# huangzh13/StyleGAN.pytorch

Hardware: AMD Instinct MI355X
Metric: img/s full G+D train step, 1024x1024 depth-9 bf16 (higher is better)
Workload: dtype bf16; 1 GPU; ffhq1024: StyleGAN 1024x1024, progressive depth index 8, logistic+R1, alpha 0.5, batch 4/GPU, global batch 4; global_batch=4, parallelism=dp1

## Files before the change

### include/sgx.h

```cpp
#ifndef SGX_H
#define SGX_H
#include <stddef.h>
#include <stdint.h>
#ifdef __cplusplus
extern "C" {
#endif

enum { SGX_F32 = 0, SGX_BF16 = 1 };
enum { SGX_ACT_NONE = 0, SGX_ACT_LRELU = 1, SGX_ACT_RELU = 2 };
enum { SGX_EINVAL = -1, SGX_EUNSUPPORTED = -2, SGX_EWORKSPACE = -3 };

int sgx_version(void);
const char* sgx_last_error(void);
int sgx_clear_error(void);
int sgx_stream_wait_stream(void* waiter, void* signaler);
int sgx_selftest_tr16(void* out256, void* stream);

int sgx_prof_start(int mode, int only_of);
int sgx_prof_count(void);
int sgx_prof_get(int i, char* name, int name_cap, float* ms, double* flops, double* bytes, char* desc, int desc_cap);

int sgx_conv3x3(const void* x, const void* w, const float* bias, void* y, int B, int H, int W, int Cin, int Cout,
                int act, const void* mask, int dtype, void* stream);
int sgx_conv4x4s2_down(const void* x, const void* w, const float* bias, void* y, int B, int H, int W, int Cin,
// ... 126 lines not shown
int sgx_sumsq_f32(const float* x, size_t n, void* ws, size_t ws_bytes, float* out, void* stream);
int sgx_scale_dev_f32(const float* x, const float* s, float alpha, float* out, size_t n, void* stream);
int sgx_logistic_loss(const float* fake, int n_fake, const float* real, int n_real, float scale, int generator, float* loss,
                      float* g_fake, float* g_real, void* stream);
size_t sgx_gemm_ws_bytes(int M, int N, int K);
int sgx_gemm_f32(const float* A, const float* Bm, float* C, int M, int N, int K, int ta, int tb, float alpha,
                 void* ws, size_t ws_bytes, void* stream);
int sgx_linear_fwd(const float* x, const float* w, const float* bias, float* y, int B, int N, int K, float w_mul, float b_mul,
                   int act, void* stream);
int sgx_linear_bwd_data(const float* gy, const float* y_act, const float* w, float* gx, int B, int N, int K, float w_mul,
                        void* stream);
int sgx_linear_bwd_param(const float* gy, const float* y_act, const float* x, float* dw, float* db, int B, int N, int K, float w_mul,
                         float b_mul, void* stream);
#define SGX_STYLE_ROW 8
int sgx_style_fwd(const float* lm, const void* table, float* y, int G, int B, int D, int total_tiles, void* stream);
int sgx_style_bwd_data(const float* gy, const void* table, float* glm, int G, int B, int D, int max_n, void* stream);
int sgx_style_bwd_param(const float* gy, const float* lm, const void* table, float* dw, float* db, int G, int B, int D,
                        int total_tiles, void* stream);

int sgx_gepi_stats(const void* x, const float* bias, const float* noise, const float* nw, float* mean, float* rstd, void* ws, size_t ws_bytes,
                   const double* pre_part, int pre_npart, int B, int HW, int C, int flags, int dtype, void* stream);
int sgx_rgb_out_epi(const void* y, const float* ebias, const float* noise, const float* nw, const float* style, const float* mean,
                    const float* rstd, const float* w, int sj, int sc, float wscale, const float* rbias, const float* low, float alpha, float beta,
                    const float* ab_dev, float* img, int B, int H, int W, int C, int dtype, void* stream);
size_t sgx_rgb_wgrad_epi_ws_bytes(int B, int HW, int C);
int sgx_rgb_wgrad_epi(const void* y, const float* g, const float* ebias, const float* noise, const float* nw, const float* style, const float* mean,
                      const float* rstd, float* dw, float* db, int sj, int sc, float scale, float bscale, void* ws, size_t ws_bytes, int B, int HW,
                      int C, int dtype, void* stream);

int sgx_adam_multi(float* const* params, const float* const* grads, float* const* exp_avg, float* const* exp_avg_sq,
                   const int64_t* sizes, int n, float beta1, float beta2, float eps, const float* step_sizes,
                   const float* bc2_sqrts, const float* grad_scale, void* stream);
int sgx_ema_multi(float* const* tgt, const float* const* src, const int64_t* sizes, int n, float beta, void* stream);
int sgx_gradnorm_clip_coef(const float* const* grads, const int64_t* sizes, int n, float max_norm, double* partial,
                           float* out, void* stream);

#ifdef __cplusplus
}
#endif
#endif
```

### stylegan/pytorch_amd/GAN.py

```python
import contextlib
import copy
import datetime
import os
import random
import time
import timeit
from collections import OrderedDict

import numpy as np
import torch
import torch.nn as nn

from . import Losses
from . import functional as F
from .Blocks import DiscriminatorBlock, DiscriminatorTop, GSynthesisBlock, InputBlock
from .CustomLayers import EqualizedConv2d, EqualizedLinear, PixelNormLayer, Truncation, act_code, apply_act
from .data import get_data_loader
from . import native
from .native import ACT_LRELU
from .optim import FusedAdam, clip_and_step, ema_update


class DeferredLoss:

    __slots__ = ("_host", "_event", "_scale", "_value", "__weakref__")

    def __init__(self, dev_scalar, scale=1.0, stream=None):
        self._scale, self._value = float(scale), None
        if dev_scalar.is_cuda:
            with torch.cuda.stream(stream) if stream is not None else contextlib.nullcontext():
                t = dev_scalar.detach().reshape(1).float()
                view, slot = native.RING.take(4)
                self._host = view.view(torch.float32)
                self._host.copy_(t, non_blocking=True)
                self._event = native.RING.mark(slot, owner=self)
        else:
            self._host, self._event = dev_scalar.detach().reshape(1).float().clone(), None

    def item(self):
        if self._value is None:
            if self._event is not None:
                self._event.synchronize()
            self._value = float(self._host[0]) * self._scale
        return self._value

    __float__ = item

    def __format__(self, spec): return format(self.item(), spec)
    def __repr__(self): return repr(self.item())
    def __add__(self, o): return self.item() + float(o)
    __radd__ = __add__
    def __sub__(self, o): return self.item() - float(o)
    def __rsub__(self, o): return float(o) - self.item()
# ... 615 lines not shown
                loss.backward()
        except BaseException:
            self._sched_abort()
            raise
        if side is not None:
            torch.cuda.current_stream().wait_stream(side)
        self._note_active_grads("d", depth)
        return loss.detach()

    def _reduce(self, kind):
        if self.dp is None:
            return
        sched = self.__dict__.pop("_sched_active", None)
        if sched is not None and not sched.recording and sched.gb is not None and sched.gb.attached():
            try:
                sched.finish()
            except RuntimeError:
                for key in [k for k, v in self.__dict__.get("_bucket_scheds", {}).items() if v is sched]:
                    self._bucket_scheds.pop(key, None)
                    self._grad_buckets.pop(key, None)
                raise
            self.__dict__["_last_sched"] = sched
            return
        gb = next((g for (k, _), g in self._grad_buckets.items() if k == kind and g.attached()), None)
        if gb is not None:
            self.dp.all_reduce_buckets(gb)
        else:
            self.dp.all_reduce_grads((self.dis if kind == "d" else self.gen).parameters())

    def _d_reduce(self):
        self._reduce("d")

    def _d_update(self):
        self.dis_optim.step()

    def _g_grads(self, noise, real_batch, depth, alpha, labels=None):
        real_samples = None
        if not isinstance(self.loss, (Losses.LogisticGAN, Losses.HingeGAN, Losses.StandardGAN, Losses.ConditionalGANLoss)):
            real_samples = self.progressive_down_sampling(real_batch, depth, alpha)
        self._wait_update("g")
        fake_samples = self.gen(noise, depth, alpha, labels)
        self._wait_update("d")
        d_all = self.__dict__.get("_sgx_dis_params")
        if d_all is None:
            d_all = self.__dict__["_sgx_dis_params"] = list(self.dis.parameters())
        d_params = [p for p in d_all if p.requires_grad]
        for p in d_params:
            p.requires_grad_(False)
        try:
            if self.conditional:
                loss = self.loss.gen_loss(real_samples, fake_samples, labels, depth, alpha)
            else:
                loss = self.loss.gen_loss(real_samples, fake_samples, depth, alpha)
            self._zero_grads("g", depth)
            side = self._param_stream()
            self._sched_begin("g", depth, side)
            try:
                with F.accumulate_param_grads(), F.param_grad_stream(side):
                    loss.backward()
            except BaseException:
                self._sched_abort()
                raise
            if side is not None:
                torch.cuda.current_stream().wait_stream(side)
            self._note_active_grads("g", depth)
        finally:
            for p in d_params:
                p.requires_grad_(True)
        return loss.detach()

    def _g_reduce(self):
        self._reduce("g")

    def _g_update(self):
        clip_and_step(self.gen_optim, max_norm=10.)
        if self.use_ema:
            self.ema_updater(self.gen_shadow, self.gen, self.ema_decay)

    def _async_update(self, kind, loss):
        upd = self.__dict__.get("_update_stream")
        if upd is None:
            upd = self.__dict__["_update_stream"] = torch.cuda.Stream(device=self.device)
        upd.wait_stream(torch.cuda.current_stream())
        with torch.cuda.stream(upd):
            (self._d_reduce if kind == "d" else self._g_reduce)()
            loss.record_stream(upd)
            loss = self.dp.all_reduce_scalar(loss)
            (self._d_update if kind == "d" else self._g_update)()
        ev = torch.cuda.Event()
        ev.record(upd)
        self.__dict__.setdefault("_pending_updates", {})[kind] = ev
        self.__dict__["_loss_stream"] = upd
        return loss

    def _wait_update(self, kind):
        ev = self.__dict__.get("_pending_updates", {}).pop(kind, None)
        if ev is not None:
            torch.cuda.current_stream().wait_event(ev)

    def _d_body(self, noise, real_batch, depth, alpha, labels=None):
        loss = self._d_grads(noise, real_batch, depth, alpha, labels)
        if self.dp is not None and not torch.cuda.is_current_stream_capturing():
            return self._async_update("d", loss)
        self._d_reduce()
        self._d_update()
        return loss

    def _g_body(self, noise, real_batch, depth, alpha, labels=None):
        loss = self._g_grads(noise, real_batch, depth, alpha, labels)
# ... 205 lines not shown
                    torch.save(self.gen.state_dict(), gen_save_file)
                    logger.info("Saving the model to: %s\n" % gen_save_file)
                    torch.save(self.dis.state_dict(), os.path.join(save_dir, "GAN_DIS_" + tag))
                    torch.save(self.gen_optim.state_dict(), os.path.join(save_dir, "GAN_GEN_OPTIM_" + tag))
                    torch.save(self.dis_optim.state_dict(), os.path.join(save_dir, "GAN_DIS_OPTIM_" + tag))
                    if self.use_ema:
                        gen_shadow_save_file = os.path.join(save_dir, "GAN_GEN_SHADOW_" + tag)
                        torch.save(self.gen_shadow.state_dict(), gen_shadow_save_file)
                        logger.info("Saving the model to: %s\n" % gen_shadow_save_file)
        logger.info('Training completed.\n')



DP_EAGER_UPDATE = os.environ.get("SGX_DP_EAGER_UPDATE", "1") != "0"


class _StepGraph:

    WARMUP = 2

    def __init__(self, sg, kind, depth):
        self.sg, self.kind, self.depth = sg, kind, int(depth)
        self.calls = 0
        self.graph = None
        self.stream = torch.cuda.Stream(device=sg.device)
        self.z = self.real = self.loss = None
        dev = sg.device
        self.ab = torch.zeros(2, dtype=torch.float32, device=dev)
        self.ab_host = torch.zeros(2, dtype=torch.float32).pin_memory()
        self.cutoff = torch.zeros(1, dtype=torch.int64, device=dev)
        self.cutoff_host = torch.zeros(1, dtype=torch.int64).pin_memory()
        self.latents2 = self.latents2_host = None
        self.adam_entries = []
        self.graph_update = None
        self.split = False
        self.done = torch.cuda.Event()

    def _mixing(self):
        gen = self.sg.gen
        return gen.training and gen.style_mixing_prob is not None and gen.style_mixing_prob > 0

    def _stage(self, noise, real_batch, alpha):
        if self.z is None:
            self.z = torch.empty_like(noise)
            self.real = torch.empty_like(real_batch)
            if self._mixing():
                self.latents2 = torch.empty_like(noise)
                self.latents2_host = torch.empty(noise.shape, dtype=noise.dtype).pin_memory()
        if self._mixing():
            l2, cut = self.sg.gen.draw_mixing_host(noise.shape, self.depth)
            native._host_copy(self.latents2_host, l2); self.cutoff_host[0] = cut
            self.latents2.copy_(self.latents2_host, non_blocking=True)
            self.cutoff.copy_(self.cutoff_host, non_blocking=True)
        self.ab_host[0] = float(alpha); self.ab_host[1] = 1.0 - float(alpha)
        self.ab.copy_(self.ab_host, non_blocking=True)
        self.z.copy_(noise); self.real.copy_(real_batch)

    def _body(self, part="all"):
        sg = self.sg
        if part == "update":
            return (sg._d_update if self.kind == "d" else sg._g_update)()
        sg.gen._mixing_override = (self.latents2, self.cutoff) if self._mixing() else None
        try:
            name = {"all": "_body", "grads": "_grads"}[part]
            return getattr(sg, "_" + self.kind + name)(self.z, self.real, self.depth, self.ab)
        finally:
# ... 14 lines not shown
            self._stage(noise, real_batch, alpha)
            loss_stream = None
            if self.graph is None and self.calls < self.WARMUP:
                loss = self._body()
                loss_stream = sg.__dict__.pop("_loss_stream", None)
            else:
                if self.graph is None:
                    err = None
                    try:
                        self._capture()
                    except Exception as e:
                        err = e
                        torch.cuda.synchronize()
                        native.lib().sgx_clear_error()
                    ok = err is None if sg.dp is None else sg.dp.all_ok(err is None)
                    if not ok:
                        import sys
                        why = f"{type(err).__name__}: {err}" if err is not None else "it failed on another rank"
                        print(f"stylegan.pytorch_amd: hipGraph capture of the {self.kind}-step failed ({why}); "
                              "continuing eagerly", file=sys.stderr)
                        self.graph = self.graph_update = None
                        self.split = False
                        sg.use_graphs = False
                        torch.cuda.synchronize()
                        self._undo_failed_capture()
                        loss = self._body()
                        out = DeferredLoss(loss, stream=sg.__dict__.pop("_loss_stream", None))
                        self.done.record()
                        self.calls += 1
                        cur.wait_stream(self.stream)
                        return out
                else:
                    FusedAdam.graph_advance(self.adam_entries)
                self.graph.replay()
                if self.split:
                    for p, g in self.grads:
                        if p.grad is not g:
                            p.grad = g
                    (sg._d_reduce if self.kind == "d" else sg._g_reduce)()
                    self.loss_global = sg.dp.all_reduce_scalar(self.loss)
                    if self.graph_update is not None:
                        self.graph_update.replay()
                    else:
                        self._body("update")
                F.bump_weight_generation(self._changed_params())
                for p, g in self.grads:
                    if p.grad is not g:
                        p.grad = g
                loss = self.loss_global if self.split else self.loss
            out = DeferredLoss(loss, stream=loss_stream)
            self.done.record()
        self.calls += 1
        cur.wait_stream(self.stream)
        return out

    def _undo_failed_capture(self):
        F.clear_pack_cache()
        for st, val in self.__dict__.pop("_adam_steps_before_capture", []):
            st["step"] = torch.tensor(val)
        sg = self.sg
        nets = [sg.dis] if self.kind == "d" else [sg.gen]
        for net in nets:
            for p in net.parameters():
                p.grad = None
        self.adam_entries = []

    def _capture(self):
        sg = self.sg
        opt = sg.dis_optim if self.kind == "d" else sg.gen_optim
        opt.ensure_state()
        self._adam_steps_before_capture = [(st, float(st["step"])) for st in opt.state.values() if "step" in st]
        native.reserve_capture_staging(1 << 20)
        F.clear_pack_cache()
        import gc
        gc_was = False
        split = sg.dp is not None
        net = sg.dis if self.kind == "d" else sg.gen
        try:
            if os.environ.get("SGX_CAPTURE_GC_GUARD", "1") != "0":
                gc.collect()
                gc_was = gc.isenabled()
                gc.disable()
            torch.cuda.synchronize()
            opt._capture_log = []
            self.graph = torch.cuda.CUDAGraph()
            with torch.cuda.graph(self.graph, stream=self.stream, capture_error_mode="relaxed"):
                self.loss = self._body("grads" if split else "all")
            self.split = split
            if split and DP_EAGER_UPDATE:
                pass
            elif split:
                self.graph_update = torch.cuda.CUDAGraph()
                with torch.cuda.graph(self.graph_update, stream=self.stream, capture_error_mode="relaxed"):
                    self._body("update")
        finally:
            self.adam_entries, opt._capture_log = (getattr(opt, "_capture_log", None) or []), None
            if gc_was:
                gc.enable()
        self.grads = [(p, p.grad) for p in net.parameters() if p.grad is not None]
```

### stylegan/pytorch_amd/functional.py

```python
import contextlib
import functools
import os
import weakref

import numpy as np
import torch
from torch.autograd import Function
from torch.autograd.function import once_differentiable

from . import native as N

_DATA_GRAD_ONLY = 0


@contextlib.contextmanager
def data_grad_only():
    global _DATA_GRAD_ONLY
    _DATA_GRAD_ONLY += 1
    try:
        yield
    finally:
        _DATA_GRAD_ONLY -= 1


# ... 138 lines not shown
    mode, _, ipad, dtype = sub
    taps = 9 if mode == "S" else 16
    O = weight.shape[0]
    return (torch.empty((taps, O, ipad), dtype=dtype, device=weight.device), torch.empty((taps, ipad, O), dtype=dtype, device=weight.device))


def _pack_mark():
    ev = torch.cuda.Event()
    ev.record()
    raw = N.stream()
    return (ev, raw, {raw})


def prepack(weights):
    rows, blk, dtype, touched = [], 0, None, []
    for w in weights:
        ent = _PACKS.get(id(w))
        if ent is None or ent[0]() is not w or not ent[3]:
            continue
        tag = _pack_tag(w)
        if ent[1] == tag:
            continue
        if w.dtype != torch.float32 or not w.is_contiguous():
            raise N.SgxError("parameters must be contiguous fp32")
        ent[1], ent[2] = tag, {}
        touched.append(ent)
        for sub in ent[3]:
            if dtype is None:
                dtype = sub[3]
            if sub[3] != dtype:
                continue
            fwd, adj = _pack_alloc(w, sub)
            ent[2][sub] = (fwd, adj)
            O, I = w.shape[0], w.shape[1]
            nb = ((O + 31) // 32) * ((sub[2] + 31) // 32)
            rows.append([w.data_ptr(), fwd.data_ptr(), adj.data_ptr(), O, I, sub[2], MODES[sub[0]],
                         int(np.float32(sub[1]).view(np.uint32)), blk, nb])
            blk += nb
    if rows:
        table, _ = N.upload(torch.tensor(rows, dtype=torch.int64), weights[0].device)
        N.check(N.lib().sgx_pack_weight_multi(N.ptr(table), len(rows), blk, N.F32 if dtype == torch.float32 else N.BF16, N.stream()),
                "sgx_pack_weight_multi")
        if not N.capturing():
            table.record_stream(torch.cuda.current_stream())
        mark = _pack_mark()
        for ent in touched:
            ent[4] = mark


def packs(weight, mode, scale, ipad, dtype):
    key = id(weight)
    ent = _PACKS.get(key)
    tag = _pack_tag(weight)
    if ent is None or ent[0]() is not weight:
        ent = [weakref.ref(weight, lambda _r, k=key: _PACKS.pop(k, None)), tag, {}, set(), None]
        _PACKS[key] = ent
    elif ent[1] != tag:
        ent[1], ent[2] = tag, {}
    sub = (mode, float(scale), int(ipad), dtype)
    ent[3].add(sub)
    got = ent[2].get(sub)
    if got is not None and ent[4] is not None:
        raw = N.stream()
        if raw not in ent[4][2] or (not _FAST_FORK and raw != ent[4][1]):
            _stream_of(raw).wait_event(ent[4][0])
            ent[4][2].add(raw)
    if got is None:
        w = _c(weight.detach())
        if w.dtype != torch.float32:
            raise N.SgxError("parameters must be fp32")
        O, I = w.shape[0], w.shape[1]
        fwd, adj = _pack_alloc(w, sub)
        N.check(N.lib().sgx_pack_weight(N.ptr(w), N.ptr(fwd), N.ptr(adj), O, I, ipad, MODES[mode], float(scale),
                                        N.F32 if dtype == torch.float32 else N.BF16, N.stream()), "sgx_pack_weight")
        got = (fwd, adj)
        ent[2][sub] = got
        ent[4] = _pack_mark()
    return got


def clear_pack_cache():
    for ent in _PACKS.values():
        ent[1], ent[2] = None, {}
    _UPBLUR_PACKS.clear()


_UPBLUR_PACKS = {}


def upblur_pack(weight, mode, scale, ipad, adjoint):
    key = (id(weight), mode, float(scale), int(ipad), bool(adjoint))
    tag = _pack_tag(weight)
    ent = _UPBLUR_PACKS.get(key)
    if ent is not None and ent[0]() is weight and ent[1] == tag:
        raw = N.stream()
        if raw not in ent[3][2] or (not _FAST_FORK and raw != ent[3][1]):
            _stream_of(raw).wait_event(ent[3][0])
            ent[3][2].add(raw)
        return ent[2]
    w = _c(weight.detach())
    if w.dtype != torch.float32 or int(ipad) != w.shape[1]:
        raise N.SgxError("conv+blur composite pack: contiguous fp32 parameter without channel padding expected")
    O, I = w.shape[0], w.shape[1]
    Nn, K = (I, O) if adjoint else (O, I)
    wc = torch.empty(((9 * 4 + 22 * 2) * Nn * K,), dtype=torch.bfloat16, device=w.device)
    N.check(N.lib().sgx_pack_upblur(N.ptr(w), N.ptr(wc), O, I, MODES[mode], int(bool(adjoint)), float(scale) / 16.0, N.stream()), "sgx_pack_upblur")
    _UPBLUR_PACKS[key] = [weakref.ref(weight, lambda _r, k=key: _UPBLUR_PACKS.pop(k, None)), tag, wc, _pack_mark()]
    return wc


@functools.lru_cache(maxsize=None)
def _splitk_ws_bytes(gi, B, H, W, Cin, Cout, dt):
    return int(N.lib().sgx_conv_splitk_ws_bytes(gi, B, H, W, Cin, Cout, dt))


def _conv_launch(geo, x, wq, bias, act, mask=None):
    B, H, W, Cin = x.shape
# ... 1841 lines not shown
```

### stylegan/pytorch_amd/native.py

```python
import ctypes
import os
import subprocess
import threading

import torch

_HERE = os.path.dirname(os.path.abspath(__file__))
LIB_PATH = os.environ.get("SGX_HIP_LIB") or os.path.join(_HERE, "libsgx_hip.so")
CSRC = os.path.join(_HERE, "csrc")

F32, BF16 = 0, 1
ACT_NONE, ACT_LRELU, ACT_RELU = 0, 1, 2
EPI_ACT, EPI_NORM = 1, 2
PACK_S, PACK_D, PACK_U, PACK_UF = 0, 1, 2, 3

_lib = None
_lock = threading.Lock()

c_void_p, c_int, c_float, c_size_t = ctypes.c_void_p, ctypes.c_int, ctypes.c_float, ctypes.c_size_t
P, I, F, Z = c_void_p, c_int, c_float, c_size_t

SIGNATURES = {
    "sgx_version": (I, []),
    "sgx_last_error": (ctypes.c_char_p, []),
# ... 66 lines not shown
    "sgx_conv4x4s2_up_blur_bits": (I, [P, P, P, P, I, I, I, I, I, I, P]),
    "sgx_pack_upblur": (I, [P, P, I, I, I, I, F, P]),
    "sgx_conv_upblur_ok": (I, [I, I, I, I, I, I]),
    "sgx_conv_upblur": (I, [P, P, P, P, I, I, I, I, I, I, P]),
    "sgx_rgbconv_ok": (I, [I, I, I, I, I]),
    "sgx_rgbconv_pack": (I, [P, F, P, F, P, F, P, P, I, P]),
    "sgx_rgbconv_fwd": (I, [P, P, P, P, P, I, I, I, I, I, I, I, P]),
    "sgx_rgbconv_tune": (I, [I, I, I]),
    "sgx_rgbconv_dgrad": (I, [P, P, P, I, I, I, I, I, P]),
    "sgx_rgbconv_wgrad_ws_bytes": (Z, [I, I, I, I]),
    "sgx_rgbconv_wgrad": (I, [P, P, I, P, F, P, F, P, F, P, P, P, P, I, P, Z, I, I, I, I, I, P]),
    "sgx_conv3x3_stats": (I, [P, P, P, P, P, P, P, Z, I, I, I, I, I, I, P]),
    "sgx_blur3x3_stats": (I, [P, P, P, P, P, P, Z, I, I, I, I, I, I, P]),
    "sgx_gepi_bwd": (I, [P, P, P, P, P, P, P, P, P, P, P, P, P, Z, I, I, I, I, I, P]),
    "sgx_pixelnorm_fwd": (I, [P, P, I, I, P]),
    "sgx_pixelnorm_bwd": (I, [P, P, P, I, I, P]),
    "sgx_mbstd_fwd": (I, [P, P, I, I, I, I, I, P]),
    "sgx_mbstd_bwd": (I, [P, P, P, I, I, I, I, I, P]),
    "sgx_mbstd_bwd2": (I, [P, P, P, P, P, I, I, I, I, I, P]),
    "sgx_sumsq_ws_bytes": (Z, []),
    "sgx_sumsq_f32": (I, [P, Z, P, Z, P, P]),
    "sgx_scale_dev_f32": (I, [P, P, F, P, Z, P]),
    "sgx_logistic_loss": (I, [P, I, P, I, F, I, P, P, P, P]),
    "sgx_gemm_ws_bytes": (Z, [I, I, I]),
    "sgx_gemm_f32": (I, [P, P, P, I, I, I, I, I, F, P, Z, P]),
    "sgx_linear_fwd": (I, [P, P, P, P, I, I, I, F, F, I, P]),
    "sgx_linear_bwd_data": (I, [P, P, P, P, I, I, I, F, P]),
    "sgx_linear_bwd_param": (I, [P, P, P, P, P, I, I, I, F, F, P]),
    "sgx_style_fwd": (I, [P, P, P, I, I, I, I, P]),
    "sgx_style_bwd_data": (I, [P, P, P, I, I, I, I, P]),
    "sgx_style_bwd_param": (I, [P, P, P, P, P, I, I, I, I, P]),
    "sgx_adam_multi": (I, [P, P, P, P, P, I, F, F, F, P, P, P, P]),
    "sgx_ema_multi": (I, [P, P, P, I, F, P]),
    "sgx_gradnorm_clip_coef": (I, [P, P, I, F, P, P, P]),
}


def build(verbose: bool = False) -> str:
    cmd = ["make", "-C", CSRC, "-j", str(min(8, os.cpu_count() or 1))]
    r = subprocess.run(cmd, capture_output=True, text=True)
    if r.returncode != 0:
        raise RuntimeError("building libsgx_hip.so failed:\n" + r.stdout[-4000:] + r.stderr[-4000:])
    if verbose:
        print(r.stdout[-2000:])
    return LIB_PATH


def lib():
    global _lib
    if _lib is None:
        with _lock:
            if _lib is None:
                if not os.path.exists(LIB_PATH):
                    raise RuntimeError(f"{LIB_PATH} is missing: run `python -c 'import __graft_entry__ as g; g.build()'` "
                                       "(there is no non-HIP fallback for this path)")
                l = ctypes.CDLL(LIB_PATH)
                for name, (res, args) in SIGNATURES.items():
                    fn = getattr(l, name)
                    fn.restype, fn.argtypes = res, args
                _lib = l
    return _lib


class SgxError(RuntimeError):
    pass

# ... 180 lines not shown
```

### stylegan/pytorch_amd/optim.py

```python
import math
from collections import OrderedDict

import torch

from . import native as N
from .functional import bump_weight_generation


_TABLES = OrderedDict()
_TABLES_MAX = 64
_GRAPH_TABLES = []
_capturing = N.capturing
_to_dev = N.upload


def _dev_i64(vals, device):
    key = (tuple(vals), str(device))
    got = _TABLES.get(key)
    if got is None:
        got = _TABLES[key] = _to_dev(torch.tensor(vals, dtype=torch.int64), device)[0]
        while len(_TABLES) > _TABLES_MAX:
            _TABLES.popitem(last=False)
    else:
        _TABLES.move_to_end(key)
    if _capturing():
        _GRAPH_TABLES.append(got)
    elif got.is_cuda:
        got.record_stream(torch.cuda.current_stream())
    return got


def _dev_f32(vals, device):
    return _to_dev(torch.tensor(vals, dtype=torch.float32), device)


class FusedAdam(torch.optim.Optimizer):

    def __init__(self, params, lr=1e-3, betas=(0.9, 0.999), eps=1e-8):
        defaults = dict(lr=lr, betas=(float(betas[0]), float(betas[1])), eps=eps, weight_decay=0, amsgrad=False,
# ... 11 lines not shown
                    st["exp_avg"] = torch.zeros_like(p, memory_format=torch.preserve_format)
                    st["exp_avg_sq"] = torch.zeros_like(p, memory_format=torch.preserve_format)

    @staticmethod
    def _bias_scalars(act, lr, b1, b2):
        steps, bc2s = [], []
        for _, st in act:
            t = float(st["step"])
            steps.append(lr / (1.0 - b1 ** t))
            bc2s.append(math.sqrt(1.0 - b2 ** t))
        return steps + bc2s

    @staticmethod
    def graph_advance(entries):
        for pinned, act, group in entries:
            for _, st in act:
                st["step"] += 1
            b1, b2 = group["betas"]
            pinned.copy_(torch.tensor(FusedAdam._bias_scalars(act, group["lr"], b1, b2), dtype=torch.float32))

    def _active(self, group):
        out = []
        for p in group["params"]:
            if p.grad is None:
                continue
            st = self.state[p]
            if len(st) == 0:
                st["step"] = torch.tensor(0.0)
                st["exp_avg"] = torch.zeros_like(p, memory_format=torch.preserve_format)
                st["exp_avg_sq"] = torch.zeros_like(p, memory_format=torch.preserve_format)
            out.append((p, st))
        return out

    @torch.no_grad()
    def step(self, closure=None, grad_scale=None):
        assert closure is None
        L = N.lib()
        changed = []
        for group in self.param_groups:
            act = self._active(group)
            if not act:
                continue
            changed.extend(p for p, _ in act)
            b1, b2 = group["betas"]
            lr, eps = group["lr"], group["eps"]
            dev = act[0][0].device
            ptrs, sizes = [[], [], [], []], []
            for p, st in act:
                g = p.grad
                if not (p.is_contiguous() and g.is_contiguous() and p.dtype == torch.float32 and g.dtype == torch.float32):
                    raise N.SgxError("FusedAdam: parameters and gradients must be contiguous fp32")
                st["step"] += 1
                ptrs[0].append(p.data_ptr()); ptrs[1].append(g.data_ptr())
                ptrs[2].append(st["exp_avg"].data_ptr()); ptrs[3].append(st["exp_avg_sq"].data_ptr())
                sizes.append(p.numel())
            n = len(act)
            table = _dev_i64(ptrs[0] + ptrs[1] + ptrs[2] + ptrs[3] + sizes, dev)
            scal, pinned = _dev_f32(self._bias_scalars(act, lr, b1, b2), dev)
            if self._capture_log is not None and _capturing():
                self._capture_log.append((pinned, act, group))
            base, sb = table.data_ptr(), scal.data_ptr()
            N.check(L.sgx_adam_multi(base, base + 8 * n, base + 16 * n, base + 24 * n, base + 32 * n, n, b1, b2, eps,
                                     sb, sb + 4 * n, None if grad_scale is None else N.ptr(grad_scale), N.stream()),
                    "sgx_adam_multi")
            if not _capturing():
                scal.record_stream(torch.cuda.current_stream())
        bump_weight_generation(changed)
        return None


@torch.no_grad()
def clip_and_step(optim: FusedAdam, max_norm: float):
    L = N.lib()
    grads = [p.grad for g in optim.param_groups for p in g["params"] if p.grad is not None]
    if not grads:
        return
    dev = grads[0].device
    n = len(grads)
    table = _dev_i64([g.data_ptr() for g in grads] + [g.numel() for g in grads], dev)
    partial = torch.empty(n * 32, dtype=torch.float64, device=dev)
    out = torch.empty(2, dtype=torch.float32, device=dev)
    N.check(L.sgx_gradnorm_clip_coef(table.data_ptr(), table.data_ptr() + 8 * n, n, float(max_norm), N.ptr(partial),
                                     N.ptr(out), N.stream()), "sgx_gradnorm_clip_coef")
    optim.step(grad_scale=out[1:])
    return out


@torch.no_grad()
def ema_update(model_tgt, model_src, beta):
    pairs = model_tgt.__dict__.get("_sgx_ema_pairs")
    if pairs is None or pairs[0] != id(model_src):
        src = dict(model_src.named_parameters())
        pairs = model_tgt.__dict__["_sgx_ema_pairs"] = (id(model_src), [(p, src[name]) for name, p in model_tgt.named_parameters()])
    tg, sr, sizes = [], [], []
    dev = None
    changed = []
    for p, q in pairs[1]:
        changed.append(p)
        assert q is not p
        if not p.is_cuda:
            raise N.SgxError("ema_update needs GPU parameters")
        tg.append(p.data_ptr()); sr.append(q.data_ptr()); sizes.append(p.numel()); dev = p.device
        assert p.is_contiguous() and q.is_contiguous()
    n = len(tg)
    table = _dev_i64(tg + sr + sizes, dev)
    base = table.data_ptr()
    N.check(N.lib().sgx_ema_multi(base, base + 8 * n, base + 16 * n, n, float(beta), N.stream()), "sgx_ema_multi")
    bump_weight_generation(changed)
```

Measured before the change: 281.6 img/s.

## Fuse Adam update with conv weight repacking and EMA in one kernel

Adds a fused optimizer path that updates Adam state for 3x3 conv weights and writes the packed forward and adjoint bf16 weight layouts plus the EMA shadow in the same kernel. Non-conv parameters get a separate fused Adam+EMA kernel. Packed weight caches are kept across graph capture and marked rebuilt, so the next forward does not have to repack them. The aim is to cut the separate repack and EMA launches and the extra passes over weight memory, at the cost of more complex cache-invalidation logic around CUDA graph replay.

After: 283.5 img/s, median of 6. About the same (+0.7%).

```diff
diff --git a/include/sgx.h b/include/sgx.h
--- a/include/sgx.h
+++ b/include/sgx.h
@@ -182,6 +182,12 @@
                    const int64_t* sizes, int n, float beta1, float beta2, float eps, const float* step_sizes,
                    const float* bc2_sqrts, const float* grad_scale, void* stream);
 int sgx_ema_multi(float* const* tgt, const float* const* src, const int64_t* sizes, int n, float beta, void* stream);
+#define SGX_ADAM_PACK_ROW 14
+#define SGX_ADAM_EMA_ROW 6
+int sgx_adam_pack_multi(const void* table, int n, int total_blocks, int dtype, float beta1, float beta2, float eps,
+                        const float* step_sizes, const float* bc2_sqrts, const float* grad_scale, float ema_beta, void* stream);
+int sgx_adam_ema_multi(const void* table, int n, float beta1, float beta2, float eps, const float* step_sizes,
+                       const float* bc2_sqrts, const float* grad_scale, float ema_beta, void* stream);
 int sgx_gradnorm_clip_coef(const float* const* grads, const int64_t* sizes, int n, float max_norm, double* partial,
                            float* out, void* stream);
 
diff --git a/stylegan/pytorch_amd/GAN.py b/stylegan/pytorch_amd/GAN.py
--- a/stylegan/pytorch_amd/GAN.py
+++ b/stylegan/pytorch_amd/GAN.py
@@ -18,7 +18,8 @@
 from .data import get_data_loader
 from . import native
 from .native import ACT_LRELU
-from .optim import FusedAdam, clip_and_step, ema_update
+from . import optim as _optim
+from .optim import FusedAdam, clip_and_step, ema_pairs, ema_update
 
 
 class DeferredLoss:
@@ -700,6 +701,7 @@
         self._reduce("d")
 
     def _d_update(self):
+        self.dis_optim.attach(packed=_conv_weights(self.dis))
         self.dis_optim.step()
 
     def _g_grads(self, noise, real_batch, depth, alpha, labels=None):
@@ -741,8 +743,10 @@
         self._reduce("g")
 
     def _g_update(self):
+        fused_ema = self.use_ema and _optim.FUSED_OPT and self.ema_updater is update_average
+        self.gen_optim.attach(packed=_conv_weights(self.gen), ema=(ema_pairs(self.gen_shadow, self.gen), self.ema_decay) if fused_ema else None)
         clip_and_step(self.gen_optim, max_norm=10.)
-        if self.use_ema:
+        if self.use_ema and not fused_ema:
             self.ema_updater(self.gen_shadow, self.gen, self.ema_decay)
 
     def _async_update(self, kind, loss):
@@ -1014,6 +1018,7 @@
         self.cutoff_host = torch.zeros(1, dtype=torch.int64).pin_memory()
         self.latents2 = self.latents2_host = None
         self.adam_entries = []
+        self.pack_deps = []
         self.graph_update = None
         self.split = False
         self.done = torch.cuda.Event()
@@ -1094,6 +1099,7 @@
                         return out
                 else:
                     FusedAdam.graph_advance(self.adam_entries)
+                F.restore_packs(self.pack_deps)
                 self.graph.replay()
                 if self.split:
                     for p, g in self.grads:
@@ -1106,6 +1112,7 @@
                     else:
                         self._body("update")
                 F.bump_weight_generation(self._changed_params())
+                F.packs_replayed(self.pack_deps)
                 for p, g in self.grads:
                     if p.grad is not g:
                         p.grad = g
@@ -1118,6 +1125,7 @@
 
     def _undo_failed_capture(self):
         F.clear_pack_cache()
+        self.pack_deps = []
         for st, val in self.__dict__.pop("_adam_steps_before_capture", []):
             st["step"] = torch.tensor(val)
         sg = self.sg
@@ -1133,7 +1141,7 @@
         opt.ensure_state()
         self._adam_steps_before_capture = [(st, float(st["step"])) for st in opt.state.values() if "step" in st]
         native.reserve_capture_staging(1 << 20)
-        F.clear_pack_cache()
+        self.pack_deps = F.clear_pack_cache(_conv_weights(sg.gen) + _conv_weights(sg.dis) if _optim.FUSED_OPT else ())
         import gc
         gc_was = False
         split = sg.dp is not None
diff --git a/stylegan/pytorch_amd/csrc/optim_pack.hip b/stylegan/pytorch_amd/csrc/optim_pack.hip
--- /dev/null
+++ b/stylegan/pytorch_amd/csrc/optim_pack.hip
@@ -0,0 +1,232 @@
+#include "common.h"
+
+__device__ __forceinline__ float adam_one(float pi, float g, float& m, float& v, float gs, float beta1, float beta2, float eps, float step_size,
+                                          float bc2_sqrt) {
+    const float gi = g * gs;
+    const float mi = beta1 * m + (1.f - beta1) * gi;
+    const float vi = beta2 * v + (1.f - beta2) * gi * gi;
+    m = mi; v = vi;
+    const float denom = sqrtf(vi) / bc2_sqrt + eps;
+    return pi - step_size * (mi / denom);
+}
+__device__ __forceinline__ float ema_one(float a, float b, float beta) { return beta * a + (1.f - beta) * b; }
+
+#define PACK_T 32
+__device__ __forceinline__ float pack_tap(const float (*raw)[PACK_T][PACK_T + 1], int r, int il, int t, int mode, float scale) {
+    if (mode == SGX_PACK_S) return scale * raw[t][r][il];
+    const int ky = t >> 2, kx = t & 3;
+    float v = 0.f;
+#pragma unroll
+    for (int a = 0; a < 2; ++a)
+#pragma unroll
+        for (int b = 0; b < 2; ++b) {
+            const int y = ky - a, x = kx - b;
+            if (y >= 0 && y < 3 && x >= 0 && x < 3) v += raw[mode == SGX_PACK_UF ? (2 - y) * 3 + (2 - x) : y * 3 + x][r][il];
+        }
+    return v * scale * (mode == SGX_PACK_D ? 0.25f : 1.f);
+}
+
+struct AdamArgs { float beta1, beta2, eps, ema_beta; };
+
+template <typename T>
+__device__ __forceinline__ void adam_pack_tile(const long long* __restrict__ row, unsigned tile, AdamArgs a, float step_size, float bc2_sqrt,
+                                               float gs) {
+    __shared__ float raw[9][PACK_T][PACK_T + 1];
+    float* __restrict__ w = reinterpret_cast<float*>(row[0]);
+    T* __restrict__ fwd = reinterpret_cast<T*>(row[1]);
+    T* __restrict__ adj = reinterpret_cast<T*>(row[2]);
+    const int O = (int)row[3], I = (int)row[4], Ip = (int)row[5], mode = (int)row[6];
+    const float scale = __uint_as_float((unsigned)row[7]);
+    const float* __restrict__ g = reinterpret_cast<const float*>(row[10]);
+    float* __restrict__ m = reinterpret_cast<float*>(row[11]);
+    float* __restrict__ v = reinterpret_cast<float*>(row[12]);
+    float* __restrict__ sh = reinterpret_cast<float*>(row[13]);
+    const int tiles_i = (Ip + PACK_T - 1) / PACK_T;
+    const int o0 = (int)(tile / tiles_i) * PACK_T, i0 = (int)(tile % tiles_i) * PACK_T;
+    const int ni = (I - i0 < PACK_T ? (I - i0 > 0 ? I - i0 : 0) : PACK_T);
+    const bool aligned = ((row[0] | row[10] | row[11] | row[12] | row[13]) & 15) == 0;
+    if (ni == PACK_T && (I * 9) % 4 == 0 && ((size_t)i0 * 9) % 4 == 0 && aligned) {
+        constexpr int PER = PACK_T * (PACK_T * 9 / 4) / 256;
+        static_assert(PER * 256 == PACK_T * (PACK_T * 9 / 4), "a tile is a whole number of 16-byte accesses per thread");
+        float4 pw[PER], pg[PER], pm[PER], pv[PER], ps[PER];
+#pragma unroll
+        for (int u = 0; u < PER; ++u) {
+            const int idx = threadIdx.x + u * 256, r = idx / (PACK_T * 9 / 4), c4 = (idx % (PACK_T * 9 / 4)) * 4;
+            const size_t at = ((size_t)(o0 + r < O ? o0 + r : O - 1) * I + i0) * 9 + c4;
+            pw[u] = *reinterpret_cast<const float4*>(w + at);
+            pg[u] = *reinterpret_cast<const float4*>(g + at);
+            pm[u] = *reinterpret_cast<const float4*>(m + at);
+            pv[u] = *reinterpret_cast<const float4*>(v + at);
+            if (sh) ps[u] = *reinterpret_cast<const float4*>(sh + at);
+        }
+#pragma unroll
+        for (int u = 0; u < PER; ++u) {
+            const int idx = threadIdx.x + u * 256, r = idx / (PACK_T * 9 / 4), c4 = (idx % (PACK_T * 9 / 4)) * 4;
+            const bool ok = o0 + r < O;
+            float e[4] = {pw[u].x, pw[u].y, pw[u].z, pw[u].w};
+            const float eg[4] = {pg[u].x, pg[u].y, pg[u].z, pg[u].w};
+            float em[4] = {pm[u].x, pm[u].y, pm[u].z, pm[u].w};
+            float ev[4] = {pv[u].x, pv[u].y, pv[u].z, pv[u].w};
+#pragma unroll
+            for (int j = 0; j < 4; ++j) e[j] = adam_one(e[j], eg[j], em[j], ev[j], gs, a.beta1, a.beta2, a.eps, step_size, bc2_sqrt);
+            if (ok) {
+                const size_t at = ((size_t)(o0 + r) * I + i0) * 9 + c4;
+                *reinterpret_cast<float4*>(w + at) = make_float4(e[0], e[1], e[2], e[3]);
+                *reinterpret_cast<float4*>(m + at) = make_float4(em[0], em[1], em[2], em[3]);
+                *reinterpret_cast<float4*>(v + at) = make_float4(ev[0], ev[1], ev[2], ev[3]);
+                if (sh) {
+                    const float es[4] = {ps[u].x, ps[u].y, ps[u].z, ps[u].w};
+                    *reinterpret_cast<float4*>(sh + at) = make_float4(ema_one(es[0], e[0], a.ema_beta), ema_one(es[1], e[1], a.ema_beta),
+                                                                      ema_one(es[2], e[2], a.ema_beta), ema_one(es[3], e[3], a.ema_beta));
+                }
+            }
+#pragma unroll
+            for (int j = 0; j < 4; ++j) raw[(c4 + j) % 9][r][(c4 + j) / 9] = ok ? e[j] : 0.f;
+        }
+    } else
+    for (int idx = threadIdx.x; idx < PACK_T * PACK_T * 9; idx += blockDim.x) {
+        const int r = idx / (PACK_T * 9), c = idx % (PACK_T * 9);
+        const int il = c / 9, k = c % 9;
+        float pn = 0.f;
+        if (o0 + r < O && il < ni) {
+            const size_t at = ((size_t)(o0 + r) * I + i0) * 9 + c;
+            float mi = m[at], vi = v[at];
+            pn = adam_one(w[at], g[at], mi, vi, gs, a.beta1, a.beta2, a.eps, step_size, bc2_sqrt);
+            w[at] = pn; m[at] = mi; v[at] = vi;
+            if (sh) sh[at] = ema_one(sh[at], pn, a.ema_beta);
+        }
+        raw[k][r][il] = pn;
+    }
+    __syncthreads();
+    const int taps = mode == SGX_PACK_S ? 9 : 16;
+    constexpr int VE = 16 / (int)sizeof(T), VPR = PACK_T / VE;
+    const bool full = (o0 + PACK_T <= O) && (i0 + PACK_T <= Ip) && (O % VE == 0) && (Ip % VE == 0);
+    if (full) {
+        for (int e = threadIdx.x; e < taps * PACK_T * VPR; e += blockDim.x) {
+            const int t = e / (PACK_T * VPR), r = (e / VPR) % PACK_T, vv = e % VPR;
+            float val[VE];
+#pragma unroll
+            for (int j = 0; j < VE; ++j) val[j] = pack_tap(raw, r, vv * VE + j, t, mode, scale);
+            VecTraits<T>::store(fwd + ((size_t)t * O + o0 + r) * Ip + i0 + vv * VE, val);
+        }
+        for (int e = threadIdx.x; e < taps * PACK_T * VPR; e += blockDim.x) {
+            const int t = e / (PACK_T * VPR), il = (e / VPR) % PACK_T, vv = e % VPR;
+            const int ta = mode == SGX_PACK_S ? 8 - t : t;
+            float val[VE];
+#pragma unroll
+            for (int j = 0; j < VE; ++j) val[j] = pack_tap(raw, vv * VE + j, il, t, mode, scale);
+            VecTraits<T>::store(adj + ((size_t)ta * Ip + i0 + il) * O + o0 + vv * VE, val);
+        }
+        return;
+    }
+    for (int e = threadIdx.x; e < taps * PACK_T * PACK_T; e += blockDim.x) {
+        const int t = e / (PACK_T * PACK_T), r = (e / PACK_T) % PACK_T, il = e % PACK_T;
+        if (o0 + r < O && i0 + il < Ip)
+            fwd[((size_t)t * O + o0 + r) * Ip + i0 + il] = from_f<T>(pack_tap(raw, r, il, t, mode, scale));
+    }
+    for (int e = threadIdx.x; e < taps * PACK_T * PACK_T; e += blockDim.x) {
+        const int t = e / (PACK_T * PACK_T), il = (e / PACK_T) % PACK_T, r = e % PACK_T;
+        const int ta = mode == SGX_PACK_S ? 8 - t : t;
+        if (o0 + r < O && i0 + il < Ip)
+            adj[((size_t)ta * Ip + i0 + il) * O + o0 + r] = from_f<T>(pack_tap(raw, r, il, t, mode, scale));
+    }
+}
+
+template <typename T>
+__global__ __launch_bounds__(256) void adam_pack_multi_kernel(const long long* __restrict__ tab, int n, AdamArgs a,
+                                                              const float* __restrict__ step_sizes, const float* __restrict__ bc2_sqrts,
+                                                              const float* __restrict__ grad_scale) {
+    int t = 0;
+    if (n <= 64) {
+        const int l = threadIdx.x & 63;
+        t = __builtin_amdgcn_readfirstlane(__popcll(__ballot(l < n && (unsigned)tab[(l < n ? l : 0) * SGX_ADAM_PACK_ROW + 8] <= blockIdx.x)) - 1);
+    } else {
+        while (t + 1 < n && (unsigned)tab[(t + 1) * SGX_ADAM_PACK_ROW + 8] <= blockIdx.x) ++t;
+    }
+    const long long* r = tab + (size_t)t * SGX_ADAM_PACK_ROW;
+    adam_pack_tile<T>(r, blockIdx.x - (unsigned)r[8], a, step_sizes[t], bc2_sqrts[t], grad_scale ? grad_scale[0] : 1.f);
+}
+
+extern "C" int sgx_adam_pack_multi(const void* table, int n, int total_blocks, int dtype, float beta1, float beta2, float eps,
+                                   const float* step_sizes, const float* bc2_sqrts, const float* grad_scale, float ema_beta, void* stream) {
+    SGX_REQUIRE(table && n > 0 && total_blocks > 0 && step_sizes && bc2_sqrts, SGX_EINVAL, "adam_pack_multi: bad args");
+    SGX_REQUIRE(dtype == SGX_F32 || dtype == SGX_BF16, SGX_EINVAL, "adam_pack_multi: bad dtype");
+    const AdamArgs a{beta1, beta2, eps, ema_beta};
+    SGX_NOTE(0.0, 0.0, "adam_pack n%d", n);
+    if (dtype == SGX_F32) hipLaunchKernelGGL(adam_pack_multi_kernel<float>, dim3((unsigned)total_blocks), dim3(256), 0, (hipStream_t)stream, (const long long*)table, n, a, step_sizes, bc2_sqrts, grad_scale);
+    else hipLaunchKernelGGL(adam_pack_multi_kernel<bf16_t>, dim3((unsigned)total_blocks), dim3(256), 0, (hipStream_t)stream, (const long long*)table, n, a, step_sizes, bc2_sqrts, grad_scale);
+    SGX_LAUNCH_CHECK("adam_pack_multi_kernel");
+    return 0;
+}
+
+#define AE_BLOCKS_X 256
+struct AdamVec {
+    float4 p, g, m, v, s;
+    __device__ __forceinline__ void load(const float* pp, const float* gg, const float* mm, const float* vv, const float* sh, int64_t i) {
+        p = reinterpret_cast<const float4*>(pp)[i]; g = reinterpret_cast<const float4*>(gg)[i];
+        m = reinterpret_cast<const float4*>(mm)[i]; v = reinterpret_cast<const float4*>(vv)[i];
+        if (sh) s = reinterpret_cast<const float4*>(sh)[i];
+    }
+    __device__ __forceinline__ void update_store(float* pp, float* mm, float* vv, float* sh, int64_t i, AdamArgs a, float step_size, float bc2_sqrt,
+                                                 float gs) {
+        float e[4] = {p.x, p.y, p.z, p.w}, em[4] = {m.x, m.y, m.z, m.w}, ev[4] = {v.x, v.y, v.z, v.w};
+        const float eg[4] = {g.x, g.y, g.z, g.w};
+#pragma unroll
+        for (int j = 0; j < 4; ++j) e[j] = adam_one(e[j], eg[j], em[j], ev[j], gs, a.beta1, a.beta2, a.eps, step_size, bc2_sqrt);
+        reinterpret_cast<float4*>(pp)[i] = make_float4(e[0], e[1], e[2], e[3]);
+        reinterpret_cast<float4*>(mm)[i] = make_float4(em[0], em[1], em[2], em[3]);
+        reinterpret_cast<float4*>(vv)[i] = make_float4(ev[0], ev[1], ev[2], ev[3]);
+        if (sh)
+            reinterpret_cast<float4*>(sh)[i] = make_float4(ema_one(s.x, e[0], a.ema_beta), ema_one(s.y, e[1], a.ema_beta),
+                                                           ema_one(s.z, e[2], a.ema_beta), ema_one(s.w, e[3], a.ema_beta));
+    }
+};
+__global__ __launch_bounds__(256) void adam_ema_multi_kernel(const long long* __restrict__ tab, AdamArgs a, const float* __restrict__ step_sizes,
+                                                             const float* __restrict__ bc2_sqrts, const float* __restrict__ grad_scale) {
+    const int t = blockIdx.y;
+    const long long* row = tab + (size_t)t * SGX_ADAM_EMA_ROW;
+    float* __restrict__ p = reinterpret_cast<float*>(row[0]);
+    const float* __restrict__ g = reinterpret_cast<const float*>(row[1]);
+    float* __restrict__ m = reinterpret_cast<float*>(row[2]);
+    float* __restrict__ v = reinterpret_cast<float*>(row[3]);
+    float* __restrict__ sh = reinterpret_cast<float*>(row[4]);
+    const int64_t n = row[5];
+    const int64_t stride = (int64_t)gridDim.x * 256;
+    int64_t i = (int64_t)blockIdx.x * 256 + threadIdx.x;
+    if (!g) {
+        for (; i < n; i += stride) sh[i] = ema_one(sh[i], p[i], a.ema_beta);
+        return;
+    }
+    const float step_size = step_sizes[t], bc2_sqrt = bc2_sqrts[t];
+    const float gs = grad_scale ? grad_scale[0] : 1.f;
+    if (((row[0] | row[1] | row[2] | row[3] | row[4]) & 15) == 0) {
+        const int64_t nv = n / 4;
+        AdamVec x, y;
+        for (; i + stride < nv; i += 2 * stride) {
+            x.load(p, g, m, v, sh, i); y.load(p, g, m, v, sh, i + stride);
+            x.update_store(p, m, v, sh, i, a, step_size, bc2_sqrt, gs); y.update_store(p, m, v, sh, i + stride, a, step_size, bc2_sqrt, gs);
+        }
+        if (i < nv) {
+            x.load(p, g, m, v, sh, i);
+            x.update_store(p, m, v, sh, i, a, step_size, bc2_sqrt, gs);
+        }
+        i = nv * 4 + (int64_t)blockIdx.x * 256 + threadIdx.x;
+    }
+    for (; i < n; i += stride) {
+        float mi = m[i], vi = v[i];
+        const float pn = adam_one(p[i], g[i], mi, vi, gs, a.beta1, a.beta2, a.eps, step_size, bc2_sqrt);
+        p[i] = pn; m[i] = mi; v[i] = vi;
+        if (sh) sh[i] = ema_one(sh[i], pn, a.ema_beta);
+    }
+}
+
+extern "C" int sgx_adam_ema_multi(const void* table, int n, float beta1, float beta2, float eps, const float* step_sizes,
+                                  const float* bc2_sqrts, const float* grad_scale, float ema_beta, void* stream) {
+    SGX_REQUIRE(table && n > 0 && n <= 65535, SGX_EINVAL, "adam_ema_multi: n=%d", n);
+    const AdamArgs a{beta1, beta2, eps, ema_beta};
+    SGX_NOTE(0.0, 0.0, "adam_ema n%d", n);
+    hipLaunchKernelGGL(adam_ema_multi_kernel, dim3(AE_BLOCKS_X, n), dim3(256), 0, (hipStream_t)stream, (const long long*)table, a, step_sizes,
+                       bc2_sqrts, grad_scale);
+    SGX_LAUNCH_CHECK("adam_ema_multi_kernel");
+    return 0;
+}
diff --git a/stylegan/pytorch_amd/functional.py b/stylegan/pytorch_amd/functional.py
--- a/stylegan/pytorch_amd/functional.py
+++ b/stylegan/pytorch_amd/functional.py
@@ -194,20 +194,71 @@
                 continue
             fwd, adj = _pack_alloc(w, sub)
             ent[2][sub] = (fwd, adj)
-            O, I = w.shape[0], w.shape[1]
-            nb = ((O + 31) // 32) * ((sub[2] + 31) // 32)
-            rows.append([w.data_ptr(), fwd.data_ptr(), adj.data_ptr(), O, I, sub[2], MODES[sub[0]],
-                         int(np.float32(sub[1]).view(np.uint32)), blk, nb])
-            blk += nb
+            rows.append(pack_row(w, sub, fwd, adj, blk))
+            blk += rows[-1][9]
     if rows:
-        table, _ = N.upload(torch.tensor(rows, dtype=torch.int64), weights[0].device)
-        N.check(N.lib().sgx_pack_weight_multi(N.ptr(table), len(rows), blk, N.F32 if dtype == torch.float32 else N.BF16, N.stream()),
-                "sgx_pack_weight_multi")
-        if not N.capturing():
-            table.record_stream(torch.cuda.current_stream())
+        _pack_multi(rows, blk, dtype, weights[0].device)
         mark = _pack_mark()
         for ent in touched:
             ent[4] = mark
+
+
+def pack_row(w, sub, fwd, adj, first_block):
+    O, I = w.shape[0], w.shape[1]
+    nb = ((O + 31) // 32) * ((sub[2] + 31) // 32)
+    return [w.data_ptr(), fwd.data_ptr(), adj.data_ptr(), O, I, sub[2], MODES[sub[0]], int(np.float32(sub[1]).view(np.uint32)), first_block, nb]
+
+
+def _pack_multi(rows, blocks, dtype, device):
+    table, _ = N.upload(torch.tensor(rows, dtype=torch.int64), device)
+    N.check(N.lib().sgx_pack_weight_multi(N.ptr(table), len(rows), blocks, N.F32 if dtype == torch.float32 else N.BF16, N.stream()),
+            "sgx_pack_weight_multi")
+    if not N.capturing():
+        table.record_stream(torch.cuda.current_stream())
+
+
+def current_packs(w):
+    ent = _PACKS.get(id(w))
+    if ent is None or ent[0]() is not w or not ent[3] or ent[1] != _pack_tag(w) or set(ent[2]) != ent[3]:
+        return None
+    return ent
+
+
+def repack_in_place(items):
+    pack_items([(w, sub, fwd, adj) for w, ent in items for sub, (fwd, adj) in ent[2].items()])
+    packs_rebuilt(items)
+
+
+def pack_items(items):
+    by_dtype = {}
+    for it in items:
+        by_dtype.setdefault(it[1][3], []).append(it)
+    for dtype, its in by_dtype.items():
+        rows, blk = [], 0
+        for w, sub, fwd, adj in its:
+            rows.append(pack_row(w, sub, fwd, adj, blk))
+            blk += rows[-1][9]
+        _pack_multi(rows, blk, dtype, its[0][0].device)
+
+
+def packs_rebuilt(items):
+    if items:
+        mark = _pack_mark()
+        for w, ent in items:
+            ent[1], ent[4] = _pack_tag(w), mark
+
+
+def restore_packs(deps):
+    stale = []
+    for w, ent, bufs in deps:
+        if ent[1] != _pack_tag(w) or any(ent[2].get(s) is not b for s, b in bufs.items()):
+            ent[2] = dict(bufs)
+            stale.append((w, ent))
+    repack_in_place(stale)
+
+
+def packs_replayed(deps):
+    packs_rebuilt([(w, ent) for w, ent, bufs in deps if ent[1] != _pack_tag(w) and all(ent[2].get(s) is b for s, b in bufs.items())])
 
 
 def packs(weight, mode, scale, ipad, dtype):
@@ -241,10 +292,17 @@
     return got
 
 
-def clear_pack_cache():
+def clear_pack_cache(keep=()):
+    kept = [(w, current_packs(w)) for w in keep]
+    kept = [(w, ent, dict(ent[2])) for w, ent in kept if ent is not None]
+    held = {id(ent) for _, ent, _ in kept}
     for ent in _PACKS.values():
-        ent[1], ent[2] = None, {}
+        if id(ent) in held:
+            ent[4] = None
+        else:
+            ent[1], ent[2] = None, {}
     _UPBLUR_PACKS.clear()
+    return kept
 
 
 _UPBLUR_PACKS = {}
diff --git a/stylegan/pytorch_amd/native.py b/stylegan/pytorch_amd/native.py
--- a/stylegan/pytorch_amd/native.py
+++ b/stylegan/pytorch_amd/native.py
@@ -122,6 +122,8 @@
     "sgx_style_bwd_param": (I, [P, P, P, P, P, I, I, I, I, P]),
     "sgx_adam_multi": (I, [P, P, P, P, P, I, F, F, F, P, P, P, P]),
     "sgx_ema_multi": (I, [P, P, P, I, F, P]),
+    "sgx_adam_pack_multi": (I, [P, I, I, I, F, F, F, P, P, P, F, P]),
+    "sgx_adam_ema_multi": (I, [P, I, F, F, F, P, P, P, F, P]),
     "sgx_gradnorm_clip_coef": (I, [P, P, I, F, P, P, P]),
 }
 
diff --git a/stylegan/pytorch_amd/optim.py b/stylegan/pytorch_amd/optim.py
--- a/stylegan/pytorch_amd/optim.py
+++ b/stylegan/pytorch_amd/optim.py
@@ -1,10 +1,13 @@
 import math
+import os
 from collections import OrderedDict
 
 import torch
 
 from . import native as N
-from .functional import bump_weight_generation
+from .functional import bump_weight_generation, current_packs, pack_items, pack_row, packs_rebuilt
+
+FUSED_OPT = os.environ.get("SGX_FUSED_OPT", "1") != "0"
 
 
 _TABLES = OrderedDict()
@@ -82,9 +85,96 @@
             out.append((p, st))
         return out
 
+    def _step_fused(self, grad_scale, packed, ema):
+        L = N.lib()
+        pairs, ema_beta = ema if ema is not None else ((), 0.0)
+        for p, q in pairs:
+            if not (p.is_cuda and p.is_contiguous() and q.is_contiguous() and p is not q):
+                raise N.SgxError("FusedAdam: the EMA needs contiguous GPU parameters")
+        shadow_of = {id(q): p for p, q in pairs}
+        packable = {id(w) for w in packed or ()}
+        groups = [(g, a) for g, a in ((g, self._active(g)) for g in self.param_groups) if a]
+        active = {id(p) for _, act in groups for p, _ in act}
+        ema_only = [(p, q) for p, q in pairs if id(q) not in active]
+        if not groups and ema_only:
+            groups = [(self.param_groups[0], [])]
+        changed, rebuilt = [p for p, _ in pairs], []
+        null = 0
+        for gi, (group, act) in enumerate(groups):
+            b1, b2 = group["betas"]
+            lr, eps = group["lr"], group["eps"]
+            tiles, rest, extra = [], [], []
+            tile_dtype = None
+            for p, st in act:
+                g = p.grad
+                if not (p.is_contiguous() and g.is_contiguous() and p.dtype == torch.float32 and g.dtype == torch.float32):
+                    raise N.SgxError("FusedAdam: parameters and gradients must be contiguous fp32")
+                st["step"] += 1
+                changed.append(p)
+                ent = current_packs(p) if id(p) in packable and p.dim() == 4 and tuple(p.shape[2:]) == (3, 3) else None
+                if ent is None:
+                    rest.append((p, st))
+                    continue
+                rebuilt.append((p, ent))
+                subs = list(ent[2].items())
+                if tile_dtype is None:
+                    tile_dtype = subs[0][0][3]
+                first = next((s for s in subs if s[0][3] == tile_dtype), None)
+                extra.extend((p, s[0]) + s[1] for s in subs if s is not first)
+                if first is None:
+                    rest.append((p, st))
+                else:
+                    tiles.append((p, st, first))
+            order = [(p, st) for p, st, _ in tiles] + rest
+            n, n1 = len(order), len(tiles)
+            dev = (order[0][0] if order else ema_only[0][0]).device
+            sb = 0
+            if n:
+                scal, pinned = _dev_f32(self._bias_scalars(order, lr, b1, b2), dev)
+                if self._capture_log is not None and _capturing():
+                    self._capture_log.append((pinned, order, group))
+                sb = scal.data_ptr()
+            gsp = None if grad_scale is None else N.ptr(grad_scale)
+            if tiles:
+                rows, blk = [], 0
+                for p, st, (sub, (fwd, adj)) in tiles:
+                    sh = shadow_of.get(id(p))
+                    rows.append(pack_row(p, sub, fwd, adj, blk) + [p.grad.data_ptr(), st["exp_avg"].data_ptr(), st["exp_avg_sq"].data_ptr(),
+                                                                  null if sh is None else sh.data_ptr()])
+                    blk += rows[-1][9]
+                table = _dev_i64([x for r in rows for x in r], dev)
+                N.check(L.sgx_adam_pack_multi(table.data_ptr(), n1, blk, N.F32 if tile_dtype == torch.float32 else N.BF16, b1, b2, eps,
+                                              sb, sb + 4 * n, gsp, float(ema_beta), N.stream()), "sgx_adam_pack_multi")
+            rows = []
+            for p, st in rest:
+                sh = shadow_of.get(id(p))
+                rows.append([p.data_ptr(), p.grad.data_ptr(), st["exp_avg"].data_ptr(), st["exp_avg_sq"].data_ptr(),
+                             null if sh is None else sh.data_ptr(), p.numel()])
+            if gi == len(groups) - 1:
+                rows.extend([q.data_ptr(), null, null, null, p.data_ptr(), p.numel()] for p, q in ema_only)
+            if rows:
+                table = _dev_i64([x for r in rows for x in r], dev)
+                N.check(L.sgx_adam_ema_multi(table.data_ptr(), len(rows), b1, b2, eps, sb + 4 * n1 if n else None,
+                                             sb + 4 * (n + n1) if n else None, gsp, float(ema_beta), N.stream()), "sgx_adam_ema_multi")
+            if n and not _capturing():
+                scal.record_stream(torch.cuda.current_stream())
+            if extra:
+                pack_items(extra)
+        bump_weight_generation(changed)
+        packs_rebuilt(rebuilt)
+        return None
+
+    _attached = (None, None)
+
+    def attach(self, packed=None, ema=None):
+        self._attached = (packed, ema)
+
     @torch.no_grad()
     def step(self, closure=None, grad_scale=None):
         assert closure is None
+        packed, ema = self._attached
+        if FUSED_OPT and (packed is not None or ema is not None):
+            return self._step_fused(grad_scale, packed, ema)
         L = N.lib()
         changed = []
         for group in self.param_groups:
@@ -136,16 +226,20 @@
     return out
 
 
-@torch.no_grad()
-def ema_update(model_tgt, model_src, beta):
+def ema_pairs(model_tgt, model_src):
     pairs = model_tgt.__dict__.get("_sgx_ema_pairs")
     if pairs is None or pairs[0] != id(model_src):
         src = dict(model_src.named_parameters())
         pairs = model_tgt.__dict__["_sgx_ema_pairs"] = (id(model_src), [(p, src[name]) for name, p in model_tgt.named_parameters()])
+    return pairs[1]
+
+
+@torch.no_grad()
+def ema_update(model_tgt, model_src, beta):
     tg, sr, sizes = [], [], []
     dev = None
     changed = []
-    for p, q in pairs[1]:
+    for p, q in ema_pairs(model_tgt, model_src):
         changed.append(p)
         assert q is not p
         if not p.is_cuda:
```
